# boolsi/boolsi

Measured on AMD Instinct MI355X. Metric: node-state-updates/s, higher is better.
Workload: dtype u32

## Files before the change

### boolsi_amd/csrc/bsx_cascade.cpp

```cpp
#include <cmath>
#include <cstdio>
#include <cstring>

#include "bsx_attract_host.h"

using namespace bsx;

namespace {
constexpr uint64_t kUnresCap = 1ull << 16;
constexpr uint64_t kNearBytes = 1ull << 32;
}

namespace bsx {

static int mirror_slots_for(bsx_handle h, uint32_t* slots_out) {
    const uint64_t entries = (h->cube_mirror ? 2 : 1) * h->journal_states;
    uint32_t slots = 64;
    while (slots < 2 * entries && slots < h->cache_lds_slots) slots *= 2;
    const size_t fixed = h->shmem + 32 + pool_extra_bytes(h->net.nw);
    while (slots < 4 * entries && slots < h->cache_lds_slots && fixed + (size_t)2 * slots * h->cache_stride <= 80 * 1024) slots *= 2;
    h->mirror_slots = *slots_out = std::min(slots, h->cache_lds_slots);
    if (h->knobs.debug) std::fprintf(stderr, "[bsx] mirror: %llu cycle states cached, %u slots\n", (unsigned long long)h->journal_states, *slots_out);
    return BSX_OK;
}

int lean_mirror_slots(bsx_handle h, uint32_t* slots_out, Totals* tot) {
    uint32_t ignored = 0;
    if (!slots_out) slots_out = &ignored;
    if (!h->journal_stale) return mirror_slots_for(h, slots_out);
    unsigned int known = 0;
    HIPCHK(h, hipMemcpy(&known, h->d_cc_count.p, sizeof(known), hipMemcpyDeviceToHost));
    if (tot) ++tot->syncs;
    known = std::min<unsigned int>(known, kCycleJournalCap);
    h->h_journal.resize(known);
    if (known) HIPCHK(h, hipMemcpy(h->h_journal.data(), h->d_cc_journal.p, known * sizeof(CycleRecord), hipMemcpyDeviceToHost));
    uint64_t states = 0;
    uint32_t taken = 0;
    for (const CycleRecord& r : h->h_journal) {
        if (taken >= (uint32_t)kTagAcc + kLdsAcc) break;
        if (!r.ready || r.length == 0 || r.length > kCycleCacheMaxLen) continue;
        states += r.length;
        ++taken;
    }
    h->journal_states = states;
    h->journal_stale = false;
    return mirror_slots_for(h, slots_out);
}

int ensure_mirror_image(bsx_handle h, AttractParams& P, size_t shmem) {
    if (!h->knobs.mirror_image) { P.mirror_image = nullptr; P.mirror_out = nullptr; return BSX_OK; }
    const size_t words = 4 + (size_t)P.cc.lds_slots * (h->cache_stride / 4);
    if (h->image_n != h->h_journal.size() || h->image_slots != P.cc.lds_slots || h->d_mirror.n < words) {
        HIPCHK(h, h->d_mirror.reserve(words));
        AttractParams B = P;
        B.count = 0;
        B.level_in = nullptr;
        B.mirror_image = nullptr;
        B.mirror_out = h->d_mirror.p;
        HIPCHK(h, launch_attract_pool((int)h->net.nw, (int)h->net.k_mux, h->lut_mode, dim3(1), shmem, h->stream, B));
        h->image_n = h->h_journal.size();
        h->image_slots = P.cc.lds_slots;
    }
    P.mirror_image = h->d_mirror.p;
    P.mirror_out = nullptr;
    return BSX_OK;
}

}

namespace {

int order_cube_digits(bsx_handle h, Cube& c) {
    const uint32_t r = (uint32_t)c.rel.size();
    if (r < 2 || r > 64 || !h->knobs.cube_order) return BSX_OK;
    uint64_t need = 0;
    for (uint32_t q = 0; q < r; ++q) need |= 1ull << c.rel[q];
    if (need & ~h->life_valid) {
        LifetimeParams L{};
        L.net = h->net;
        for (int w = 0; w < kMaxW32; ++w) { L.fixmask[w] = h->sp.fixmask[w]; L.fixval[w] = h->sp.fixval[w]; L.base[w] = c.base[w]; L.free_mask[w] = c.free_mask[w]; }
        L.n_digits = r;
        for (uint32_t q = 0; q < r; ++q) L.node[q] = h->model.any[c.rel[q]];
        HIPCHK(h, h->d_life.reserve(64));
        HIPCHK(h, hipMemsetAsync(h->d_life.p, 0, 64 * sizeof(uint32_t), h->stream));
        L.out = h->d_life.p;
        HIPCHK(h, launch_digit_lifetimes((int)h->net.nw, (int)h->net.k_mux, h->lut_mode, h->shmem, h->stream, L));
        uint32_t measured[64];
        HIPCHK(h, hipMemcpyAsync(measured, h->d_life.p, sizeof(measured), hipMemcpyDeviceToHost, h->stream));
        HIPCHK(h, hipStreamSynchronize(h->stream));
        for (uint32_t q = 0; q < r; ++q) h->life_cache[c.rel[q]] = measured[q];
        h->life_valid |= need;
    }
    uint32_t life[64];
    for (uint32_t q = 0; q < r; ++q) life[q] = h->life_cache[c.rel[q]];
// ... 191 lines not shown
            }
        }
        const size_t shmem_here = Q.lower_build ? h->shmem + (size_t)B.slots * h->cache_stride + 32 + pool_lower_extra_bytes(nw) : B.shmem;
        hipStream_t const st = i == 0 ? main_st : tail_st;
        HIPCHK(h, launch_attract_pool((int)nw, (int)h->net.k_mux, h->lut_mode, grid, shmem_here, st, Q));
        if (i == 0) HIPCHK(h, hipEventRecord(ev[1], main_st));
        if (i == 0 && side) HIPCHK(h, hipStreamWaitEvent(tail_st, ev[1], 0));
    }
    if (side) {
        HIPCHK(h, hipEventRecord(ev[2], tail_st));
        slot_busy[slot] = ev[2];
    }
    return BSX_OK;
}

int evaluate_chain(bsx_handle h, const CascadeEnv& env, const CascadeShape& sh, const Chain& ch, MergedTable& pass_table,
                   u128& pass_none, u128& pass_ref, int& verdict, uint32_t& lower_to) {
    const AttractParams& P = env.P;
    Totals& tot = env.tot;
    const uint64_t max_t = env.max_t, max_len = env.max_len;
    const uint32_t nw = h->net.nw, rec_words = nw + 3;
    verdict = kChainOk;
    uint64_t n_entries = 0;
    for (uint32_t i = 0; i < ch.top; ++i) {
        const ChainLevel& l = ch.lv[i];
        const Counters& c = h->ctr_seen[ch.ctr_base + i];
        const uint64_t classes = i == 0 ? 1ull << l.k_bits : n_entries << l.k_bits;
        if (i > 0 && n_entries == 0) break;
        tot.steps_exec += c.steps_exec;
        if (h->knobs.debug)
            std::fprintf(stderr, "[bsx] cube 2^%u (%u digits free) at digit value %llu%s: depth %u%s, %u digits here (%u relevant), %llu classes, %llu near a cycle, %llu unresolved\n",
                         ch.c1.a, ch.c1.n_free, (unsigned long long)ch.c1.d_lo, ch.c1.fix_mask ? " [sub-block]" : "", l.depth, i == 0 ? " (top)" : l.per_parent ? " (per parent)" : "", l.k_bits, l.r_here,
                         (unsigned long long)classes, (unsigned long long)c.near_classes, (unsigned long long)c.straggler_classes);
        if (h->knobs.debug && l.per_parent) {
            const LeafProgram& prog = h->h_leaf[ch.index];
            std::fprintf(stderr, "[bsx] per-parent level: kb %u, %u enumerated rules, %u free rules, m %u\n", prog.kb, prog.n_enum, prog.n_free, prog.m);
        }
        if (c.straggler_overflow) { verdict = kChainGiveUp; return BSX_OK; }
        if (c.near_overflow) { verdict = kChainLower; lower_to = l.depth - 1; return BSX_OK; }
        n_entries = c.near_classes;
        {
            double* seen = h->plan.near_seen[i == 0 ? 0 : 1][std::min<uint32_t>(l.depth, kMaxCubeLevels)];
            seen[0] += (double)classes; seen[1] += (double)c.near_classes;
        }
        const uint32_t us = l.unit_shift;
        merge_cube_counters(pass_table, c, us, nw);
        fold_cube_level(c, us, max_t, pass_none, pass_ref);
        const uint64_t n_unres = c.straggler_classes;
        if (!n_unres) continue;
        if (n_unres > kUnresCap) { verdict = kChainGiveUp; return BSX_OK; }
        std::vector<uint32_t> recs(n_unres * rec_words);
        HIPCHK(h, hipMemcpy(recs.data(), h->d_unres.p + (size_t)(ch.ctr_base + i) * kUnresCap * rec_words, recs.size() * 4, hipMemcpyDeviceToHost));
        ++tot.syncs;
        std::vector<uint32_t> st(n_unres * nw);
        for (uint64_t q = 0; q < n_unres; ++q) std::copy(recs.begin() + q * rec_words, recs.begin() + q * rec_words + nw, st.begin() + q * nw);
        DevBuf<uint32_t> d_states;
        DevBuf<ProblemRec32> d_res;
        HIPCHK(h, d_states.upload(st));
        HIPCHK(h, d_res.alloc(n_unres));
        AttractParams S = P;
        S.sp = l.cube.sp;
        S.sp.tp_origin = 0;
        S.count = n_unres;
        S.states = d_states.p;
        S.per_problem = d_res.p;
        S.max_len = BSX_T_INF;
// ... 244 lines not shown
```

### boolsi_amd/csrc/bsx_device.h

```cpp
#pragma once
#include <cstddef>
#include <stdint.h>

namespace bsx {

constexpr int kWave = 64;
constexpr int kBlock = 512;
constexpr int kWavesPerBlock = kBlock / kWave;
constexpr int kPoolBlockThreads = 768;
constexpr uint32_t kPoolCap = 112;
constexpr uint32_t kPoolSlots = 128;
constexpr uint32_t pool_rec_words(uint32_t nw) { return nw + 4; }
constexpr uint32_t kLowerFoundWords = 256;
constexpr int kMaxW32 = 8;
constexpr int kMaxMuxK = 6;
constexpr int kTableSlots = 64;
constexpr uint32_t kStepLimit = 1u << 30;
constexpr uint64_t kDigestSeed = 0xCBF29CE484222325ull;
constexpr uint64_t kDigestPrime = 0x100000001B3ull;
constexpr uint32_t kMaxDepositRuns = 64;

struct DevNet {
    uint32_t n_nodes;
    uint32_t nw;
// ... 29 lines not shown
    uint64_t first_variant;
};

struct LogRec {
    uint32_t key[kMaxW32];
    uint32_t length;
    uint32_t pad;
    uint64_t count;
    uint64_t sum_l;
    uint64_t sum_l2_lo, sum_l2_hi;
};
static_assert(sizeof(LogRec) == 72, "LogRec layout");

struct ProblemRec32 {
    uint32_t key[kMaxW32];
    uint32_t length;
    uint32_t trajectory_l;
    uint32_t found;
    uint32_t pad;
};

struct alignas(256) Counters {
    unsigned long long cursor;
    unsigned long long steps_ref;
    unsigned long long steps_exec;
    unsigned long long n_none;
    unsigned long long log_cursor;
    unsigned int log_overflow;
    unsigned int step_limit_hits;
    unsigned long long n_stragglers;
    unsigned long long n_cache_resolved;
    unsigned long long straggler_classes;
    unsigned int straggler_overflow;
    unsigned int pad;
    unsigned long long table_inserts;
    unsigned int table_overflow;
    unsigned int near_overflow;
    unsigned long long phase_sum[3];
    unsigned long long phase_max[3];
    unsigned long long acc_cnt[64], acc_sl[64], acc_sl2_lo[64], acc_sl2_hi[64];
    unsigned int acc_len[64];
    unsigned int acc_key[64][kMaxW32];
    unsigned long long fix_cnt[64], fix_sl[64], fix_sl2[64];
    unsigned long long fix_none, fix_ref, fix_capfail;
    unsigned long long near_classes;
    unsigned long long t_first_not, t_last;
    unsigned long long wave_iters;
    unsigned long long service_rounds;
    unsigned long long diag[4];
};

constexpr uint32_t kCycleCacheMaxLen = 64;
constexpr uint32_t kCycleCacheLdsBytes = 16 * 1024;
constexpr uint32_t kCycleJournalCap = 4096;
constexpr uint32_t kCycleClaimSlots = 8192;
constexpr int kTagAcc = 3;
constexpr uint32_t kLdsAcc = 61;
constexpr uint32_t kMergeGroup = 32;
constexpr uint32_t kMergeSlots = 256;
constexpr uint32_t lean_acc_bytes(uint32_t nw) { return (kTagAcc + kLdsAcc) * (8 + 8 + 4 + 4 + 4 * nw) + 16 + kWavesPerBlock * (kMergeSlots + 256); }

struct CycleRecord {
    uint32_t key[kMaxW32];
    uint32_t length;
    uint32_t ready;
};
static_assert(sizeof(CycleRecord) == 40, "CycleRecord layout");

struct CycleCache {
    CycleRecord* journal;
    unsigned int* journal_count;
    unsigned int* claims;
    uint32_t enabled;
    uint32_t lds_slots;
};

struct LevelDesc {
    unsigned long long n_entries;
    unsigned int abort;
    unsigned int pad;
};
constexpr uint32_t kMaxCubeLevels = 16;
constexpr uint32_t kSideStreams = 4;
constexpr uint32_t kMaxChains = 48;
constexpr uint32_t kMaxChainBlocks = 160;
constexpr size_t kLevelDescBytes = 3584;
constexpr size_t kPublishTicketOffset = kLevelDescBytes - 16;
static_assert(sizeof(LevelDesc) * (kMaxChainBlocks + kMaxChains + 1) <= kPublishTicketOffset && kLevelDescBytes % 256 == 0, "descriptor block");

constexpr uint32_t kLeafMaxDeps = 64;
constexpr uint32_t kLeafMaxBits = 14;
constexpr uint32_t kLeafMaxK = 4;
struct LeafDep {
// ... 144 lines not shown
```

### boolsi_amd/csrc/bsx_engine.h

```cpp
#pragma once
#include <hip/hip_runtime.h>

#include <map>
#include <string>
#include <utility>
#include <vector>

#include "bsx.h"
#include "bsx_device.h"
#include "bsx_knobs.h"
#include "bsx_model.h"

namespace bsx {

struct WideHost;

template <typename T>
struct DevBuf {
    T* p = nullptr;
    size_t n = 0;
    DevBuf() = default;
    DevBuf(const DevBuf&) = delete;
    DevBuf& operator=(const DevBuf&) = delete;
    ~DevBuf() { release(); }
// ... 32 lines not shown

    bool have_net = false;
    uint32_t n_nodes = 0, w64 = 0;
    bsx::DevNet net{};
    int lut_mode = 0;
    size_t shmem = 0;
    size_t shmem_attract = 0;

    bool cache_enabled = true;
    int lean_blocks_per_cu = 0;
    bool fast_ok = true;
    bool pool_ok = false;
    size_t cache_stride = 0;
    std::vector<bsx::CycleRecord> h_journal;
    bool journal_stale = true;
    uint32_t mirror_slots = 64;
    uint64_t journal_states = 0;
    bool cube_mirror = false;
    uint32_t fast_steps = 0;
    bool fast_calibrated = false;
    uint32_t cache_lds_slots = 0;
    bsx::DevBuf<bsx::CycleRecord> d_cc_journal;
    bsx::DevBuf<unsigned int> d_cc_claims;
    bsx::DevBuf<unsigned int> d_cc_count;

    bsx::DevBuf<bsx::LogRec> d_log;
    bsx::DevBuf<bsx::LogRec> d_table;
    uint64_t table_slots = 0;
    bool table_dirty = false;
    bsx::DevBuf<uint32_t> d_strag;
    bsx::DevBuf<uint32_t> d_mirror;
    size_t image_n = ~size_t(0);
    uint32_t image_slots = 0;
    bsx::DevBuf<uint32_t> d_near_seg[bsx::kSideStreams];
    bsx::DevBuf<uint32_t> d_near_list[bsx::kSideStreams][2];
    hipStream_t side[bsx::kSideStreams] = {};
    bsx::DevBuf<uint32_t> d_unres;
    bsx::DevBuf<bsx::LeafProgram> d_leaf;
    bsx::LeafProgram* h_leaf = nullptr;
    uint32_t life_cache[64] = {};
    uint64_t life_valid = 0;
    bsx::PlanState plan;
    bsx::DevBuf<uint32_t> d_life;
    bsx::DevBuf<uint32_t> d_lut, d_masks, d_wide_desc, d_wide_preds, d_wide_tt;

    bsx::HostModel model;

    bool have_space = false;
    uint64_t variant_count = 1;
    bool variant_count_saturated = false;
    uint32_t tp_max = 0;
    bsx::DevSpace sp{};
    bsx::DevBuf<uint32_t> d_any, d_fv, d_pv, d_set, d_clr;

    bsx::DevBuf<unsigned char> d_ctr_raw;
    bsx::LevelDesc* d_level = nullptr;
    bsx::Counters* d_ctr = nullptr;
    bsx::Counters* h_ctr = nullptr;
    volatile uint32_t* h_flag = nullptr;
    uint32_t flag_seq = 0;
    hipEvent_t ev_top0 = nullptr, ev_top1 = nullptr;
    std::vector<bsx::Counters> ctr_seen;
    std::vector<hipEvent_t> ev_chain;
    hipStream_t aux[8] = {};
    hipEvent_t aux_done[8] = {};
    bsx::DevBuf<bsx::Counters> d_ctr_multi;
// ... 54 lines not shown
```

### boolsi_amd/csrc/bsx_kernels_common.h

```cpp
#pragma once
#include <hip/hip_runtime.h>
#include <type_traits>
#include "bsx_device.h"

namespace bsx {

__device__ __forceinline__ uint32_t bfi(uint32_t sel, uint32_t a, uint32_t b) {
    uint32_t r;
    asm("v_bfi_b32 %0, %1, %2, %3" : "=v"(r) : "v"(sel), "v"(a), "v"(b));
    return r;
}

#define BSX_KERNARG(Type, name)                                                                          \
    const Type* name = (const Type*)__builtin_amdgcn_kernarg_segment_ptr();                              \
    asm volatile("" : "+s"(name))

__device__ __forceinline__ uint32_t rank_below(uint64_t mask) {
    return __builtin_amdgcn_mbcnt_hi((uint32_t)(mask >> 32), __builtin_amdgcn_mbcnt_lo((uint32_t)mask, 0u));
}

template <int NW>
__device__ __forceinline__ bool eq_words(const uint32_t (&a)[NW], const uint32_t (&b)[NW]) {
    uint32_t d = 0;
#pragma unroll
// ... 286 lines not shown
        else { digit = (uint32_t)(variant & 1); variant >>= 1; }
        const int st = digit_state(range, digit);
        if (st >= 0) { put_bit<NW>(pr.fm, node, 1); put_bit<NW>(pr.fv, node, (uint32_t)st); }
    }
    pr.pv_digits = 0;
    pr.tp = sp.tp_origin;
    for (uint32_t j = 0; j < sp.n_pv; ++j) {
        const uint32_t t = sp.pv[3 * j], range = sp.pv[3 * j + 2];
        uint32_t digit;
        if (range == 3) { digit = (uint32_t)(variant % 3); variant /= 3; }
        else { digit = (uint32_t)(variant & 1); variant >>= 1; }
        pr.pv_digits |= (uint64_t)digit << (2 * j);
        if (digit_state(range, digit) >= 0 && t > pr.tp) pr.tp = t;
    }
}

template <int NW>
__device__ __forceinline__ void apply_perturbations(const DevSpace& sp, uint32_t t, uint64_t pv_digits,
                                                    uint32_t (&s)[NW]) {
    if (t <= sp.tp_origin) {
#pragma unroll
        for (int w = 0; w < NW; ++w)
            s[w] = (s[w] & ~sp.sched_clr[t * NW + w]) | sp.sched_set[t * NW + w];
    }
    for (uint32_t j = 0; j < sp.n_pv; ++j) {
        if (sp.pv[3 * j] == t) {
            const int st = digit_state(sp.pv[3 * j + 2], (uint32_t)(pv_digits >> (2 * j)) & 3u);
            if (st >= 0) put_bit<NW>(s, sp.pv[3 * j + 1], (uint32_t)st);
        }
    }
}

template <int NW, int K, int LM>
__device__ __forceinline__ NetView<NW, K, LM> stage_network(const DevNet& net, uint32_t* smem, uint32_t*& smem_free) {
    constexpr bool LDS_LUT = LM != kLutGlobal;
    NetView<NW, K, LM> nv;
    if constexpr (LDS_LUT) {
        if ((uint32_t)(uintptr_t)(__attribute__((address_space(3))) uint32_t*)smem != 0u) __builtin_trap();
    }
    uint32_t* p = smem;
    uint32_t* smasks = p;
    const uint32_t n_masks = (1u << K) * NW;
    for (uint32_t i = threadIdx.x; i < n_masks; i += blockDim.x) smasks[i] = net.masks[i];
    p += (n_masks + 3u) & ~3u;
    if (LDS_LUT) {
        uint32_t* slut = p;
        const uint4* src = reinterpret_cast<const uint4*>(net.lut);
        uint4* dst = reinterpret_cast<uint4*>(slut);
        const uint32_t n4 = net.lut_words >> 2;
        for (uint32_t i = threadIdx.x; i < n4; i += blockDim.x) dst[i] = src[i];
        p += net.lut_words;
        nv.lut = slut;
    } else {
        nv.lut = net.lut;
    }
    __syncthreads();
    nv.masks = smasks;
    if constexpr (NetView<NW, K, LM>::kMasksInRegs) {
#pragma unroll
        for (int i = 0; i < (1 << K) * NW; ++i) nv.mreg[i] = smasks[i];
    } else {
        nv.mreg[0] = 0;
    }
    nv.n_wide = net.n_wide;
    nv.wide_desc = net.wide_desc;
    nv.wide_preds = net.wide_preds;
    nv.wide_tt = net.wide_tt;
    smem_free = p;
    return nv;
}

__device__ __forceinline__ uint32_t digest_ybit(uint32_t t) { return (t * 0x9E3779B1u) >> 31; }
template <int NW>
__device__ __forceinline__ uint64_t digest_fold_words(uint64_t dg, const uint32_t (&s)[NW], uint32_t w64) {
#pragma unroll
    for (int w = 0; w < (NW + 1) / 2; ++w) {
        uint64_t word = s[2 * w];
        if (2 * w + 1 < NW) word |= (uint64_t)s[2 * w + 1] << 32;
        if ((uint32_t)w < w64) dg = (dg ^ word) * kDigestPrime;
    }
    return dg;
}

__device__ __forceinline__ uint64_t bcast64(uint64_t v, int src_lane) {
    const uint32_t lo = __builtin_amdgcn_readlane((uint32_t)v, src_lane);
    const uint32_t hi = __builtin_amdgcn_readlane((uint32_t)(v >> 32), src_lane);
    return ((uint64_t)hi << 32) | lo;
}

__device__ __forceinline__ unsigned long long wave_sum(unsigned long long v) {
#pragma unroll
    for (int off = 32; off >= 1; off >>= 1) {
        const uint32_t lo = __shfl_xor((uint32_t)v, off, 64);
        const uint32_t hi = __shfl_xor((uint32_t)(v >> 32), off, 64);
        v += ((unsigned long long)hi << 32) | lo;
    }
    return v;
}
__device__ __forceinline__ void wave_atomic_add(unsigned long long* dst, unsigned long long v, int lane) {
    const unsigned long long total = wave_sum(v);
    if (lane == 0 && total) atomicAdd(dst, total);
}
// ... 341 lines not shown
```

### boolsi_amd/csrc/bsx_pool_kernel.h

```cpp
#pragma once
#include "bsx_kernels_common.h"
#include "bsx_leaf.h"

namespace bsx {

constexpr int kPoolBlock = kPoolBlockThreads;
constexpr int kPoolWaves = kPoolBlock / 64;
constexpr uint32_t kPoolGroup = 64;

constexpr int pool_min_waves(int nw) { return nw <= 2 ? 6 : 2; }

#define BSX_RARE_PARAMS(name) BSX_KERNARG(AttractParams, name)

template <int NW>
__device__ __forceinline__ void deposit_runs(const DevSpace& sp, uint64_t d, uint32_t (&s)[NW], uint32_t run_first = 0,
                                             uint32_t run_end = 0xFFFFFFFFu) {
    const uint32_t end = run_end < sp.n_runs ? run_end : sp.n_runs;
    for (uint32_t r = run_first; r < end; ++r) {
        const uint32_t desc = sp.deposit[2 * r], mask = sp.deposit[2 * r + 1];
        const uint32_t piece = ((uint32_t)(d >> (desc & 63u)) & mask) << ((desc >> 16) & 31u);
        const uint32_t word = (desc >> 8) & 7u;
#pragma unroll
        for (int w = 0; w < NW; ++w) s[w] |= (word == (uint32_t)w) ? piece : 0u;
    }
}

template <int NW, int K, int LM, bool CUBE, bool LOWER = false>
__global__ __launch_bounds__(kPoolBlock, pool_min_waves(NW)) void k_attract_pool(const AttractParams P) {
    static_assert(CUBE || !LOWER, "the lower-level build is a cube build");
    extern __shared__ __attribute__((aligned(16))) uint32_t smem[];
    uint32_t* smem_free;
#ifdef BSX_DIAG
    const unsigned long long dbg_t0 = wall_clock64();
#endif
    uint64_t n_items = P.count, chunk_first = P.chunk_first;
    uint32_t chunk = P.chunk;
    if constexpr (CUBE) {
        if (P.level_in) {
            const unsigned long long listed = P.level_in->n_entries;
            n_items = P.level_in->abort ? 0ull : listed << P.entry_shift;
            if constexpr (LOWER) {
                if (P.leaf && n_items) n_items = ((listed + 63ull) & ~63ull) * leaf_parts(P.leaf->m, listed, (uint64_t)gridDim.x * kPoolWaves);
            }
            if (n_items == 0) return;
            const uint64_t n_waves = (uint64_t)gridDim.x * kPoolWaves;
            if (n_items < (1ull << 28)) { chunk_first = ((n_items + n_waves - 1) / n_waves + 63) / 64 * 64; chunk = 0; }
            else { chunk_first = 4096; chunk = 4096; }
            if ((uint64_t)blockIdx.x * chunk_first >= n_items) return;
        }
    }
    if constexpr (CUBE) {
        if (threadIdx.x == 0 && !P.mirror_out) atomicMax(&P.ctr->t_first_not, ~(unsigned long long)wall_clock64());
    }
    const NetView<NW, K, LM> nv = stage_network<NW, K, LM>(P.net, smem, smem_free);
    const uint32_t lane = threadIdx.x & 63, wave = __builtin_amdgcn_readfirstlane(threadIdx.x >> 6);
    const uint32_t tp = P.sp.tp_origin;
    const bool has_warmup = tp != 0;
    const bool counting = CUBE || P.merge >= 2;
    constexpr bool cube = CUBE;
    const int32_t fast_steps = (int32_t)P.fast_steps;
    const uint32_t cmask = P.cc.lds_slots - 1;
    constexpr int S = CacheLayout<NW>::kStride;
    constexpr uint32_t kAccs = (uint32_t)kTagAcc + kLdsAcc;
    constexpr uint32_t R = cube ? NW + 2 : pool_rec_words(NW);
    constexpr uint32_t kCap = cube ? (kPoolCap * pool_rec_words(NW)) / (NW + 2) : kPoolCap;

    uint32_t* lc = smem + (((uint32_t)(smem_free - smem) + 3u) & ~3u);
    const uint32_t lc_words = kCacheHeaderWords + P.cc.lds_slots * S;
    unsigned long long* acc_sl2 = reinterpret_cast<unsigned long long*>(lc + ((lc_words + 1u) & ~1u));
    unsigned long long* acc_sl2h = acc_sl2 + kAccs;
    unsigned long long* acc_sl = acc_sl2h + kAccs;
    unsigned long long* acc_cnt = acc_sl + kAccs;
    uint32_t* lamtab = reinterpret_cast<uint32_t*>(acc_cnt + kAccs);
    uint32_t* keytab = lamtab + kAccs;
    constexpr uint32_t kWaveWords = LOWER ? 0u : kPoolCap * pool_rec_words(NW) + 128 + kPoolSlots / 4;
    constexpr uint32_t kFoundWords = LOWER ? kLowerFoundWords : 0u;
    constexpr uint32_t kLowerCntWords = LOWER ? 2u * kAccs : 0u;
    static_assert(kAccs % 2 == 0 && kWaveWords % 2 == 0, "64-bit LDS atomics need 8-byte aligned tables");
    unsigned long long* wg_ctr = reinterpret_cast<unsigned long long*>(keytab + ((kAccs * NW + 1u) & ~1u));
    uint32_t* midtab = reinterpret_cast<uint32_t*>(wg_ctr + 4);
    uint32_t* wave_base = midtab + 64 * NW + kFoundWords + wave * (kWaveWords + kLowerCntWords);
    typedef volatile uint32_t __attribute__((address_space(3))) lds_vu32;
    typedef volatile uint8_t __attribute__((address_space(3))) lds_vu8;
    lds_vu32* const pool = (lds_vu32*)(__attribute__((address_space(3))) uint32_t*)wave_base;
    lds_vu32* const dd_acc = pool + kPoolCap * pool_rec_words(NW);
    lds_vu8* const dd_ids = (lds_vu8*)(dd_acc + 128);

    uint32_t fm0[NW], fv0[NW];
    uint32_t any_fixed = 0;
#pragma unroll
    for (int w = 0; w < NW; ++w) { fm0[w] = P.sp.fixmask[w]; fv0[w] = P.sp.fixval[w]; any_fixed |= fm0[w]; }
    const bool has_fixed = any_fixed != 0;
    const uint32_t* const image = P.mirror_image;
    if (image) { for (uint32_t i = threadIdx.x; i < lc_words; i += blockDim.x) lc[i] = image[i]; }
    else { for (uint32_t i = threadIdx.x; i < lc_words; i += blockDim.x) lc[i] = 0; }
    for (uint32_t i = threadIdx.x; i < kAccs; i += blockDim.x) { acc_sl2[i] = 0; acc_sl2h[i] = 0; acc_sl[i] = 0; acc_cnt[i] = 0; lamtab[i] = 0; }
    if (threadIdx.x < 4) wg_ctr[threadIdx.x] = 0;
    if constexpr (!LOWER) { dd_acc[2 * lane] = 0; dd_acc[2 * lane + 1] = 0; }
    else { wave_base[lane] = 0; wave_base[64 + lane] = 0; }
    __syncthreads();
    if (!image && threadIdx.x == 0) {
        uint32_t seen = 0, n_states = 0, n_attr = 0;
        cache_pull<NW, K>(P.cc, nv, fm0, fv0, lc, seen, n_states, n_attr, kAccs);
    }
    __syncthreads();
    if (P.mirror_out) {
        for (uint32_t i = threadIdx.x; i < lc_words; i += blockDim.x) P.mirror_out[i] = lc[i];
        return;
    }
    const uint32_t* cbase = lc + kCacheHeaderWords;
    for (uint32_t sl = threadIdx.x; sl < P.cc.lds_slots; sl += blockDim.x) {
        const uint32_t tg = cbase[sl * S + NW] & kTagMask;
        if (tg) {
            lamtab[tg - 1] = cbase[sl * S + NW + 1];
#pragma unroll
            for (int w = 0; w < NW; ++w) keytab[(tg - 1) * NW + w] = cbase[sl * S + NW + 2 + w];
        }
    }
    __syncthreads();
    if constexpr (cube) {
        for (uint32_t i = threadIdx.x; i < 64u; i += blockDim.x) {
            uint32_t m[NW];
#pragma unroll
            for (int w = 0; w < NW; ++w) m[w] = 0;
            deposit_runs<NW>(P.sp, (uint64_t)i << 6, m, 6u, 12u);
#pragma unroll
            for (int w = 0; w < NW; ++w) midtab[i * NW + w] = m[w];
        }
    }
    const uint32_t depth = (cube && P.cube_depth > 1u) ? P.cube_depth : 1u;
    const bool from_entries = cube && P.entries != nullptr;
    if constexpr (cube) {
        if (threadIdx.x == 0) { lc[1] = 0; lc[2] = 0; }
        __syncthreads();
        if (depth == 1u && !has_warmup) {
            constexpr uint32_t kFoundCap = LOWER ? kLowerFoundWords : kCap * R;
            auto inside = [&](uint32_t sl) -> bool {
                const uint32_t* e = cbase + sl * S;
                const uint32_t tw = e[NW];
                if ((tw & kTagMask) == 0 || (tw & kTagRep)) return false;
                uint32_t outside = 0;
#pragma unroll
                for (int w = 0; w < NW; ++w) outside |= (e[w] ^ P.sp.origin[w]) & ~P.cube_free[w];
                return outside == 0;
            };
            lds_vu32* const found0 = (lds_vu32*)(__attribute__((address_space(3))) uint32_t*)(midtab + 64 * NW);
            for (uint32_t sl = threadIdx.x; sl < P.cc.lds_slots; sl += blockDim.x) {
                if (!inside(sl)) continue;
                const uint32_t at = atomicAdd((uint32_t*)(__attribute__((address_space(3))) uint32_t*)&lc[1], 1u);
                if (at < kFoundCap) found0[at] = sl;
            }
            __syncthreads();
            if (threadIdx.x == 0) {
                const uint32_t n_in = lc[1];
                auto add_rep = [&](uint32_t sl) {
                    const uint32_t* e = cbase + sl * S;
                    uint32_t rep[NW], key[NW], differs = 0;
#pragma unroll
                    for (int w = 0; w < NW; ++w) {
                        rep[w] = e[w] & ~P.cube_umask[w];
                        differs |= rep[w] ^ e[w];
                        key[w] = e[NW + 2 + w];
                    }
                    if (differs) cache_insert_lds<NW>(lc, cmask, rep, e[NW + 1], key, (e[NW] & kTagMask) | kTagRep);
                };
                if (n_in <= kFoundCap) {
                    for (uint32_t i = 0; i < n_in; ++i) add_rep(found0[i]);
                } else {
                    for (uint32_t sl = 0; sl < P.cc.lds_slots; ++sl) if (inside(sl)) add_rep(sl);
                }
            }
        }
    }
    __syncthreads();
    const bool t0_lookup = cube && !has_warmup && depth == 1u && __builtin_amdgcn_readfirstlane(lc[1]) != 0;
    uint32_t lane_part[NW];
#pragma unroll
    for (int w = 0; w < NW; ++w) lane_part[w] = 0;
    if constexpr (cube) deposit_runs<NW>(P.sp, (uint64_t)lane, lane_part);
    uint32_t u_hi[NW];
    uint64_t u_hi_tag = ~0ull;
#pragma unroll
    for (int w = 0; w < NW; ++w) u_hi[w] = 0;

    const uint32_t cap_rel = (P.cap_rel_inf || P.max_t - tp >= (kStepLimit / 4)) ? 0xFFFFFFFFu : (uint32_t)(P.max_t - tp);

    using cnt_t = std::conditional_t<CUBE, unsigned long long, uint32_t>;
    uint32_t nexec = 0;
    const uint64_t first_dyn = (uint64_t)gridDim.x * kPoolWaves * chunk_first;
    WaveQueue q{0, 0, chunk != 0 && n_items > first_dyn};
    {
        const uint64_t b = ((uint64_t)wave * gridDim.x + blockIdx.x) * chunk_first;
        if (b < n_items) { q.next = b; q.end = (b + chunk_first < n_items) ? b + chunk_first : n_items; }
    }
    uint32_t head = 0, count = 0;
#ifdef BSX_DIAG
    unsigned long long dbg_iters = 0, dbg_fresh = 0, dbg_fresh_keep = 0, dbg_pool_in = 0, dbg_pool_keep = 0, dbg_merged = 0;
    bool dbg_is_fresh = false;
#endif

    uint32_t ptag = 0;
    auto fresh_state = [&](uint64_t pos, bool lv, uint32_t (&S0)[NW]) {
        if ((pos >> 12) != u_hi_tag) {
            u_hi_tag = pos >> 12;
#pragma unroll
            for (int w = 0; w < NW; ++w) u_hi[w] = P.sp.origin[w];
            deposit_runs<NW>(P.sp, pos & ~0xFFFull, u_hi, 12u);
// ... 595 lines not shown
                if constexpr (NW == 2) {
                    typedef volatile bsx_u32x4 __attribute__((address_space(3))) lds_v4;
                    bsx_u32x4 v;
                    v.x = A[0]; v.y = A[1]; v.z = mlo; v.w = packed;
                    *(lds_v4*)(pool + r) = v;
                } else {
#pragma unroll
                    for (int w = 0; w < NW; ++w) pool[r + w] = A[w];
                    pool[r + NW] = mlo; pool[r + NW + 1] = packed;
                }
            } else if constexpr (NW % 2 == 0) {
                typedef volatile bsx_u32x2 __attribute__((address_space(3))) lds_v2;
                lds_v2* rec = (lds_v2*)(pool + r);
#pragma unroll
                for (int w = 0; w < NW; w += 2) { bsx_u32x2 v; v.x = A[w]; v.y = A[w + 1]; rec[w / 2] = v; }
                bsx_u32x2 b0, b1;
                b0.x = base; b0.y = mlo; b1.x = mhi; b1.y = (uint32_t)t;
                rec[NW / 2] = b0; rec[NW / 2 + 1] = b1;
            } else {
#pragma unroll
                for (int w = 0; w < NW; ++w) pool[r + w] = A[w];
                pool[r + NW] = base; pool[r + NW + 1] = mlo; pool[r + NW + 2] = mhi; pool[r + NW + 3] = (uint32_t)t;
            }
        }
        count += (uint32_t)__popcll(keepers);
        __builtin_amdgcn_fence(__ATOMIC_RELEASE, "wavefront");
        __builtin_amdgcn_wave_barrier();
    }

    __syncthreads();
#ifdef BSX_DIAG
    const unsigned long long dbg_t2 = wall_clock64();
#endif
    static_assert(kAccs == 64, "one lane per accumulator");
    if (wave == 0) {
        const uint32_t a = lane;
        const unsigned long long cn = acc_cnt[a];
        const uint64_t nb = __ballot(cn != 0);
        if (nb) {
            unsigned long long at0 = 0;
            if (!cube && lane == 0) at0 = atomicAdd(&P.ctr->log_cursor, (unsigned long long)__popcll(nb));
            const unsigned long long at = bcast64(at0, 0) + rank_below(nb);
            if (cn) {
                const unsigned long long sl = acc_sl[a];
                if constexpr (cube) {
                    Counters* c = P.ctr;
                    atomicAdd(&c->acc_cnt[a], cn);
                    atomicAdd(&c->acc_sl[a], sl);
                    const unsigned long long lo = acc_sl2[a];
                    const unsigned long long old = atomicAdd(&c->acc_sl2_lo[a], lo);
                    const unsigned long long up = acc_sl2h[a] + ((old + lo < old) ? 1ull : 0ull);
                    if (up) atomicAdd(&c->acc_sl2_hi[a], up);
                    c->acc_len[a] = lamtab[a];
#pragma unroll
                    for (int w = 0; w < NW; ++w) c->acc_key[a][w] = keytab[a * NW + w];
                } else if (at < P.log_cap) {
                    LogRec r;
#pragma unroll
                    for (int w = 0; w < kMaxW32; ++w) r.key[w] = 0;
#pragma unroll
                    for (int w = 0; w < NW; ++w) r.key[w] = keytab[a * NW + w];
                    r.length = lamtab[a]; r.pad = 0; r.count = cn; r.sum_l = sl; r.sum_l2_lo = acc_sl2[a]; r.sum_l2_hi = acc_sl2h[a];
                    P.log[at] = r;
                } else {
                    atomicOr(&P.ctr->log_overflow, 1u);
                }
                atomicAdd(&wg_ctr[2], sl + cn * lamtab[a]);
            }
        }
    }
#ifdef BSX_DIAG
    if (lane == 0) {
        atomicAdd(&P.ctr->wave_iters, dbg_iters); atomicAdd(&P.ctr->service_rounds, dbg_fresh);
        atomicAdd(&P.ctr->diag[0], dbg_fresh_keep); atomicAdd(&P.ctr->diag[1], dbg_pool_in);
        atomicAdd(&P.ctr->diag[2], dbg_pool_keep); atomicAdd(&P.ctr->diag[3], dbg_merged);
    }
    if (threadIdx.x == 0) {
        const unsigned long long dbg_t3 = wall_clock64();
        atomicAdd(&P.ctr->phase_sum[0], dbg_t1 - dbg_t0); atomicMax(&P.ctr->phase_max[0], dbg_t1 - dbg_t0);
        atomicAdd(&P.ctr->phase_sum[1], dbg_t2 - dbg_t1); atomicMax(&P.ctr->phase_max[1], dbg_t2 - dbg_t1);
        atomicAdd(&P.ctr->phase_sum[2], dbg_t3 - dbg_t2); atomicMax(&P.ctr->phase_max[2], dbg_t3 - dbg_t2);
    }
#endif
    {
        const unsigned long long w_exec = wave_sum((unsigned long long)nexec);
        if (lane == 0 && w_exec) atomicAdd(&wg_ctr[3], w_exec);
    }
    __builtin_amdgcn_fence(__ATOMIC_RELEASE, "workgroup");
    __builtin_amdgcn_s_barrier();
    __builtin_amdgcn_fence(__ATOMIC_ACQUIRE, "workgroup");
    if (threadIdx.x == 0) {
        if constexpr (cube) {
            BSX_RARE_PARAMS(Pr);
            if (Pr->level_out) {
                const uint32_t listed = lc[2];
                const uint32_t mine = listed < Pr->near_cap ? listed : (uint32_t)Pr->near_cap;
                lc[1] = mine ? (uint32_t)atomicAdd(&Pr->level_out->n_entries, (unsigned long long)mine) : 0u;
                if (listed) atomicAdd(&P.ctr->near_classes, (unsigned long long)listed);
                if (listed > Pr->near_cap) {
                    atomicOr(&Pr->level_out->abort, 1u);
                    atomicOr(&P.ctr->near_overflow, 1u);
                }
            }
        }
        const unsigned long long ref = wg_ctr[2] + (P.cap_rel_inf ? 0ull : wg_ctr[1] * P.max_t);
        if (ref) atomicAdd(&P.ctr->steps_ref, ref);
        if (wg_ctr[3]) atomicAdd(&P.ctr->steps_exec, wg_ctr[3]);
        if (wg_ctr[0]) atomicAdd(&P.ctr->n_none, wg_ctr[0]);
        if constexpr (cube) atomicMax(&P.ctr->t_last, (unsigned long long)wall_clock64());
    }
    if constexpr (cube) {
        BSX_RARE_PARAMS(Pr);
        if (Pr->level_out) {
            __syncthreads();
            const uint32_t listed = lc[2], base = lc[1];
            const uint64_t words = (uint64_t)(listed < Pr->near_cap ? listed : (uint32_t)Pr->near_cap) * (NW + 1);
            const uint32_t* src = Pr->near + (uint64_t)blockIdx.x * Pr->near_cap * (NW + 1);
            uint32_t* dst = Pr->near_list + (uint64_t)base * (NW + 1);
            for (uint64_t i = threadIdx.x; i < words; i += kPoolBlock) dst[i] = src[i];
        }
    }
}

template <int NW, int K, int LM>
__global__ __launch_bounds__(1024) void k_digit_lifetimes(const LifetimeParams P) {
    extern __shared__ __attribute__((aligned(16))) uint32_t smem[];
    uint32_t* smem_free;
    const NetView<NW, K, LM> nv = stage_network<NW, K, LM>(P.net, smem, smem_free);
    const uint32_t digit = threadIdx.x / kLifeTrials, trial = threadIdx.x % kLifeTrials;
    if (digit >= P.n_digits) return;
    uint32_t fm[NW], fv[NW], x[NW], y[NW];
    uint32_t any_fixed = 0;
    const uint32_t node = P.node[digit];
#pragma unroll
    for (int w = 0; w < NW; ++w) {
        fm[w] = P.fixmask[w]; fv[w] = P.fixval[w]; any_fixed |= fm[w];
        uint32_t rnd = (trial * 0x9E3779B1u + (uint32_t)w * 0x85EBCA6Bu + 0x27D4EB2Fu) * 0xC2B2AE35u;
        rnd ^= rnd >> 15; rnd *= 0x2C1B3C6Du; rnd ^= rnd >> 12;
        const uint32_t bit = ((node >> 5) == (uint32_t)w) ? 1u << (node & 31) : 0u;
        x[w] = (P.base[w] | (trial ? rnd & P.free_mask[w] : 0u)) & ~bit;
        y[w] = x[w] | bit;
    }
    uint32_t t = 0;
    while (t < kLifeSteps && !eq_words<NW>(x, y)) {
        uint32_t nx[NW], ny[NW];
        net_step<NW, K>(nv, x, fm, fv, nx, any_fixed != 0);
        net_step<NW, K>(nv, y, fm, fv, ny, any_fixed != 0);
// ... 113 lines not shown
```

Baseline: 3583 billion.

## Stage whole LDS prologue from a precomputed image and move near-list reservation earlier

The mirror image now holds the full LDS prologue (masks, LUT, cycle cache, accumulators, lamtab, keytab, counters), not just the cache. When an image is present, each workgroup loads it with one batched vector copy instead of staging the network, zeroing accumulators and rebuilding lookup tables, which removes several barriers. The near-list slot reservation atomic moves earlier to wave 1 so the final barrier before the copy-out can go. This adds image-size bookkeeping and depends on the LDS layout matching pool_image_words exactly, which is a correctness risk.

```diff
diff --git a/boolsi_amd/csrc/bsx_cascade.cpp b/boolsi_amd/csrc/bsx_cascade.cpp
--- a/boolsi_amd/csrc/bsx_cascade.cpp
+++ b/boolsi_amd/csrc/bsx_cascade.cpp
@@ -49,8 +49,8 @@
 
 int ensure_mirror_image(bsx_handle h, AttractParams& P, size_t shmem) {
     if (!h->knobs.mirror_image) { P.mirror_image = nullptr; P.mirror_out = nullptr; return BSX_OK; }
-    const size_t words = 4 + (size_t)P.cc.lds_slots * (h->cache_stride / 4);
-    if (h->image_n != h->h_journal.size() || h->image_slots != P.cc.lds_slots || h->d_mirror.n < words) {
+    const size_t words = pool_image_words(h->net.nw, h->net.k_mux, h->lut_mode != 0, h->net.lut_words, P.cc.lds_slots);
+    if (h->image_n != h->h_journal.size() || h->image_slots != P.cc.lds_slots || h->image_words != words || h->d_mirror.n < words) {
         HIPCHK(h, h->d_mirror.reserve(words));
         AttractParams B = P;
         B.count = 0;
@@ -60,6 +60,7 @@
         HIPCHK(h, launch_attract_pool((int)h->net.nw, (int)h->net.k_mux, h->lut_mode, dim3(1), shmem, h->stream, B));
         h->image_n = h->h_journal.size();
         h->image_slots = P.cc.lds_slots;
+        h->image_words = words;
     }
     P.mirror_image = h->d_mirror.p;
     P.mirror_out = nullptr;
@@ -317,6 +318,11 @@
             std::fprintf(stderr, "[bsx] cube 2^%u (%u digits free) at digit value %llu%s: depth %u%s, %u digits here (%u relevant), %llu classes, %llu near a cycle, %llu unresolved\n",
                          ch.c1.a, ch.c1.n_free, (unsigned long long)ch.c1.d_lo, ch.c1.fix_mask ? " [sub-block]" : "", l.depth, i == 0 ? " (top)" : l.per_parent ? " (per parent)" : "", l.k_bits, l.r_here,
                          (unsigned long long)classes, (unsigned long long)c.near_classes, (unsigned long long)c.straggler_classes);
+        if (h->knobs.debug && c.phase_wgs)
+            std::fprintf(stderr, "[bsx]   diag: depth %u, %llu classes, %u workgroups with work; prologue / loop / epilogue, us: mean %.1f / %.1f / %.1f, slowest %.1f / %.1f / %.1f\n",
+                         l.depth, (unsigned long long)classes, c.phase_wgs,
+                         c.phase_sum[0] / 100.0 / c.phase_wgs, c.phase_sum[1] / 100.0 / c.phase_wgs, c.phase_sum[2] / 100.0 / c.phase_wgs,
+                         c.phase_max[0] / 100.0, c.phase_max[1] / 100.0, c.phase_max[2] / 100.0);
         if (h->knobs.debug && l.per_parent) {
             const LeafProgram& prog = h->h_leaf[ch.index];
             std::fprintf(stderr, "[bsx] per-parent level: kb %u, %u enumerated rules, %u free rules, m %u\n", prog.kb, prog.n_enum, prog.n_free, prog.m);
diff --git a/boolsi_amd/csrc/bsx_device.h b/boolsi_amd/csrc/bsx_device.h
--- a/boolsi_amd/csrc/bsx_device.h
+++ b/boolsi_amd/csrc/bsx_device.h
@@ -85,7 +85,7 @@
     unsigned long long n_cache_resolved;
     unsigned long long straggler_classes;
     unsigned int straggler_overflow;
-    unsigned int pad;
+    unsigned int phase_wgs;
     unsigned long long table_inserts;
     unsigned int table_overflow;
     unsigned int near_overflow;
@@ -112,6 +112,18 @@
 constexpr uint32_t kMergeGroup = 32;
 constexpr uint32_t kMergeSlots = 256;
 constexpr uint32_t lean_acc_bytes(uint32_t nw) { return (kTagAcc + kLdsAcc) * (8 + 8 + 4 + 4 + 4 * nw) + 16 + kWavesPerBlock * (kMergeSlots + 256); }
+
+constexpr uint32_t pool_image_words(uint32_t nw, uint32_t k_mux, bool lut_in_lds, uint32_t lut_words, uint32_t lds_slots) {
+    const uint32_t accs = (uint32_t)kTagAcc + kLdsAcc;
+    const uint32_t masks = (((1u << k_mux) * nw) + 3u) & ~3u;
+    const uint32_t lut = lut_in_lds ? lut_words : 0u;
+    const uint32_t mirror = 4u + lds_slots * (((2u * nw + 2u) + 3u) & ~3u);
+    const uint32_t sums = 4u * 2u * accs;
+    const uint32_t lamtab = accs;
+    const uint32_t keytab = (accs * nw + 1u) & ~1u;
+    const uint32_t wg_ctr = 4u * 2u;
+    return (masks + lut + mirror + sums + lamtab + keytab + wg_ctr + 3u) & ~3u;
+}
 
 struct CycleRecord {
     uint32_t key[kMaxW32];
diff --git a/boolsi_amd/csrc/bsx_engine.h b/boolsi_amd/csrc/bsx_engine.h
--- a/boolsi_amd/csrc/bsx_engine.h
+++ b/boolsi_amd/csrc/bsx_engine.h
@@ -88,6 +88,7 @@
     bsx::DevBuf<uint32_t> d_mirror;
     size_t image_n = ~size_t(0);
     uint32_t image_slots = 0;
+    size_t image_words = 0;
     bsx::DevBuf<uint32_t> d_near_seg[bsx::kSideStreams];
     bsx::DevBuf<uint32_t> d_near_list[bsx::kSideStreams][2];
     hipStream_t side[bsx::kSideStreams] = {};
diff --git a/boolsi_amd/csrc/bsx_kernels_common.h b/boolsi_amd/csrc/bsx_kernels_common.h
--- a/boolsi_amd/csrc/bsx_kernels_common.h
+++ b/boolsi_amd/csrc/bsx_kernels_common.h
@@ -342,42 +342,75 @@
 }
 
 template <int NW, int K, int LM>
-__device__ __forceinline__ NetView<NW, K, LM> stage_network(const DevNet& net, uint32_t* smem, uint32_t*& smem_free) {
+__device__ __forceinline__ NetView<NW, K, LM> network_view(const DevNet& net, uint32_t* smem, uint32_t*& smem_free) {
     constexpr bool LDS_LUT = LM != kLutGlobal;
     NetView<NW, K, LM> nv;
     if constexpr (LDS_LUT) {
         if ((uint32_t)(uintptr_t)(__attribute__((address_space(3))) uint32_t*)smem != 0u) __builtin_trap();
     }
     uint32_t* p = smem;
-    uint32_t* smasks = p;
-    const uint32_t n_masks = (1u << K) * NW;
-    for (uint32_t i = threadIdx.x; i < n_masks; i += blockDim.x) smasks[i] = net.masks[i];
-    p += (n_masks + 3u) & ~3u;
+    nv.masks = p;
+    p += (((1u << K) * NW) + 3u) & ~3u;
     if (LDS_LUT) {
-        uint32_t* slut = p;
-        const uint4* src = reinterpret_cast<const uint4*>(net.lut);
-        uint4* dst = reinterpret_cast<uint4*>(slut);
-        const uint32_t n4 = net.lut_words >> 2;
-        for (uint32_t i = threadIdx.x; i < n4; i += blockDim.x) dst[i] = src[i];
+        nv.lut = p;
         p += net.lut_words;
-        nv.lut = slut;
     } else {
         nv.lut = net.lut;
     }
-    __syncthreads();
-    nv.masks = smasks;
-    if constexpr (NetView<NW, K, LM>::kMasksInRegs) {
-#pragma unroll
-        for (int i = 0; i < (1 << K) * NW; ++i) nv.mreg[i] = smasks[i];
-    } else {
-        nv.mreg[0] = 0;
-    }
+    nv.mreg[0] = 0;
     nv.n_wide = net.n_wide;
     nv.wide_desc = net.wide_desc;
     nv.wide_preds = net.wide_preds;
     nv.wide_tt = net.wide_tt;
     smem_free = p;
     return nv;
+}
+
+template <int NW, int K, int LM>
+__device__ __forceinline__ void load_mask_regs(NetView<NW, K, LM>& nv) {
+    if constexpr (NetView<NW, K, LM>::kMasksInRegs) {
+#pragma unroll
+        for (int i = 0; i < (1 << K) * NW; ++i) nv.mreg[i] = nv.masks[i];
+    }
+}
+
+template <int NW, int K, int LM>
+__device__ __forceinline__ NetView<NW, K, LM> stage_network(const DevNet& net, uint32_t* smem, uint32_t*& smem_free) {
+    constexpr bool LDS_LUT = LM != kLutGlobal;
+    NetView<NW, K, LM> nv = network_view<NW, K, LM>(net, smem, smem_free);
+    uint32_t* smasks = smem;
+    const uint32_t n_masks = (1u << K) * NW;
+    for (uint32_t i = threadIdx.x; i < n_masks; i += blockDim.x) smasks[i] = net.masks[i];
+    if (LDS_LUT) {
+        const uint4* src = reinterpret_cast<const uint4*>(net.lut);
+        uint4* dst = reinterpret_cast<uint4*>(smem + ((n_masks + 3u) & ~3u));
+        const uint32_t n4 = net.lut_words >> 2;
+        for (uint32_t i = threadIdx.x; i < n4; i += blockDim.x) dst[i] = src[i];
+    }
+    __syncthreads();
+    load_mask_regs<NW, K, LM>(nv);
+    return nv;
+}
+
+constexpr int kImageLoadsPerRound = 4;
+__device__ __forceinline__ void copy_table_image(uint32_t* smem, const uint32_t* image, uint32_t n4) {
+    const bsx_u32x4* src = reinterpret_cast<const bsx_u32x4*>(__builtin_assume_aligned(image, 16));
+    bsx_u32x4* dst = reinterpret_cast<bsx_u32x4*>(__builtin_assume_aligned(smem, 16));
+    static_assert(kImageLoadsPerRound == 4, "the round's loads are pinned by name below");
+    for (uint32_t first = threadIdx.x; first < n4; first += kImageLoadsPerRound * blockDim.x) {
+        bsx_u32x4 v[kImageLoadsPerRound];
+#pragma unroll
+        for (int j = 0; j < kImageLoadsPerRound; ++j) {
+            const uint32_t i = first + (uint32_t)j * blockDim.x;
+            v[j] = src[i < n4 ? i : n4 - 1u];
+        }
+        asm volatile("" : "+v"(v[0]), "+v"(v[1]), "+v"(v[2]), "+v"(v[3]));
+#pragma unroll
+        for (int j = 0; j < kImageLoadsPerRound; ++j) {
+            const uint32_t i = first + (uint32_t)j * blockDim.x;
+            if (i < n4) dst[i] = v[j];
+        }
+    }
 }
 
 __device__ __forceinline__ uint32_t digest_ybit(uint32_t t) { return (t * 0x9E3779B1u) >> 31; }
diff --git a/boolsi_amd/csrc/bsx_pool_kernel.h b/boolsi_amd/csrc/bsx_pool_kernel.h
--- a/boolsi_amd/csrc/bsx_pool_kernel.h
+++ b/boolsi_amd/csrc/bsx_pool_kernel.h
@@ -52,7 +52,8 @@
     if constexpr (CUBE) {
         if (threadIdx.x == 0 && !P.mirror_out) atomicMax(&P.ctr->t_first_not, ~(unsigned long long)wall_clock64());
     }
-    const NetView<NW, K, LM> nv = stage_network<NW, K, LM>(P.net, smem, smem_free);
+    const uint32_t* const image = P.mirror_image;
+    NetView<NW, K, LM> nv = image ? network_view<NW, K, LM>(P.net, smem, smem_free) : stage_network<NW, K, LM>(P.net, smem, smem_free);
     const uint32_t lane = threadIdx.x & 63, wave = __builtin_amdgcn_readfirstlane(threadIdx.x >> 6);
     const uint32_t tp = P.sp.tp_origin;
     const bool has_warmup = tp != 0;
@@ -91,49 +92,64 @@
 #pragma unroll
     for (int w = 0; w < NW; ++w) { fm0[w] = P.sp.fixmask[w]; fv0[w] = P.sp.fixval[w]; any_fixed |= fm0[w]; }
     const bool has_fixed = any_fixed != 0;
-    const uint32_t* const image = P.mirror_image;
-    if (image) { for (uint32_t i = threadIdx.x; i < lc_words; i += blockDim.x) lc[i] = image[i]; }
-    else { for (uint32_t i = threadIdx.x; i < lc_words; i += blockDim.x) lc[i] = 0; }
-    for (uint32_t i = threadIdx.x; i < kAccs; i += blockDim.x) { acc_sl2[i] = 0; acc_sl2h[i] = 0; acc_sl[i] = 0; acc_cnt[i] = 0; lamtab[i] = 0; }
-    if (threadIdx.x < 4) wg_ctr[threadIdx.x] = 0;
-    if constexpr (!LOWER) { dd_acc[2 * lane] = 0; dd_acc[2 * lane + 1] = 0; }
-    else { wave_base[lane] = 0; wave_base[64 + lane] = 0; }
-    __syncthreads();
-    if (!image && threadIdx.x == 0) {
-        uint32_t seen = 0, n_states = 0, n_attr = 0;
-        cache_pull<NW, K>(P.cc, nv, fm0, fv0, lc, seen, n_states, n_attr, kAccs);
-    }
-    __syncthreads();
-    if (P.mirror_out) {
-        for (uint32_t i = threadIdx.x; i < lc_words; i += blockDim.x) P.mirror_out[i] = lc[i];
-        return;
-    }
     const uint32_t* cbase = lc + kCacheHeaderWords;
-    for (uint32_t sl = threadIdx.x; sl < P.cc.lds_slots; sl += blockDim.x) {
-        const uint32_t tg = cbase[sl * S + NW] & kTagMask;
-        if (tg) {
-            lamtab[tg - 1] = cbase[sl * S + NW + 1];
-#pragma unroll
-            for (int w = 0; w < NW; ++w) keytab[(tg - 1) * NW + w] = cbase[sl * S + NW + 2 + w];
-        }
-    }
-    __syncthreads();
-    if constexpr (cube) {
-        for (uint32_t i = threadIdx.x; i < 64u; i += blockDim.x) {
-            uint32_t m[NW];
-#pragma unroll
-            for (int w = 0; w < NW; ++w) m[w] = 0;
-            deposit_runs<NW>(P.sp, (uint64_t)i << 6, m, 6u, 12u);
-#pragma unroll
-            for (int w = 0; w < NW; ++w) midtab[i * NW + w] = m[w];
+    auto launch_tables = [&]() {
+        if constexpr (!LOWER) { dd_acc[2 * lane] = 0; dd_acc[2 * lane + 1] = 0; }
+        else { wave_base[lane] = 0; wave_base[64 + lane] = 0; }
+        if constexpr (cube) {
+            for (uint32_t i = threadIdx.x; i < 64u; i += blockDim.x) {
+                uint32_t m[NW];
+#pragma unroll
+                for (int w = 0; w < NW; ++w) m[w] = 0;
+                deposit_runs<NW>(P.sp, (uint64_t)i << 6, m, 6u, 12u);
+#pragma unroll
+                for (int w = 0; w < NW; ++w) midtab[i * NW + w] = m[w];
+            }
+        }
+    };
+    if (image) {
+        copy_table_image(smem, image, pool_image_words(NW, K, LM != kLutGlobal, P.net.lut_words, P.cc.lds_slots) >> 2);
+        launch_tables();
+        __syncthreads();
+        load_mask_regs<NW, K, LM>(nv);
+    } else {
+        for (uint32_t i = threadIdx.x; i < lc_words; i += blockDim.x) lc[i] = 0;
+        for (uint32_t i = threadIdx.x; i < kAccs; i += blockDim.x) { acc_sl2[i] = 0; acc_sl2h[i] = 0; acc_sl[i] = 0; acc_cnt[i] = 0; lamtab[i] = 0; }
+        if (threadIdx.x < 4) wg_ctr[threadIdx.x] = 0;
+        if (P.mirror_out) for (uint32_t i = threadIdx.x; i < ((kAccs * NW + 1u) & ~1u); i += blockDim.x) keytab[i] = 0;
+        __syncthreads();
+        if (threadIdx.x == 0) {
+            uint32_t seen = 0, n_states = 0, n_attr = 0;
+            cache_pull<NW, K>(P.cc, nv, fm0, fv0, lc, seen, n_states, n_attr, kAccs);
+        }
+        __syncthreads();
+        for (uint32_t sl = threadIdx.x; sl < P.cc.lds_slots; sl += blockDim.x) {
+            const uint32_t tg = cbase[sl * S + NW] & kTagMask;
+            if (tg) {
+                lamtab[tg - 1] = cbase[sl * S + NW + 1];
+#pragma unroll
+                for (int w = 0; w < NW; ++w) keytab[(tg - 1) * NW + w] = cbase[sl * S + NW + 2 + w];
+            }
+        }
+        __syncthreads();
+        if (P.mirror_out) {
+            const uint32_t n4 = pool_image_words(NW, K, LM != kLutGlobal, P.net.lut_words, P.cc.lds_slots) >> 2;
+            const uint4* src = reinterpret_cast<const uint4*>(smem);
+            uint4* dst = reinterpret_cast<uint4*>(P.mirror_out);
+            for (uint32_t i = threadIdx.x; i < n4; i += blockDim.x) dst[i] = src[i];
+            return;
+        }
+        launch_tables();
+        if constexpr (cube) {
+            if (threadIdx.x == 0) { lc[1] = 0; lc[2] = 0; }
+            __syncthreads();
         }
     }
     const uint32_t depth = (cube && P.cube_depth > 1u) ? P.cube_depth : 1u;
     const bool from_entries = cube && P.entries != nullptr;
+    const bool rep_search = cube && depth == 1u && !has_warmup;
     if constexpr (cube) {
-        if (threadIdx.x == 0) { lc[1] = 0; lc[2] = 0; }
-        __syncthreads();
-        if (depth == 1u && !has_warmup) {
+        if (rep_search) {
             constexpr uint32_t kFoundCap = LOWER ? kLowerFoundWords : kCap * R;
             auto inside = [&](uint32_t sl) -> bool {
                 const uint32_t* e = cbase + sl * S;
@@ -172,7 +188,7 @@
             }
         }
     }
-    __syncthreads();
+    if (!image || rep_search) __syncthreads();
     const bool t0_lookup = cube && !has_warmup && depth == 1u && __builtin_amdgcn_readfirstlane(lc[1]) != 0;
     uint32_t lane_part[NW];
 #pragma unroll
@@ -834,6 +850,19 @@
 #ifdef BSX_DIAG
     const unsigned long long dbg_t2 = wall_clock64();
 #endif
+    static_assert(kPoolWaves >= 2, "the span is reserved by wave 1");
+    if constexpr (cube) {
+        if (threadIdx.x == 64) {
+            BSX_RARE_PARAMS(Pr);
+            LevelDesc* const out = Pr->level_out;
+            const uint64_t cap = Pr->near_cap;
+            if (out) {
+                const uint32_t listed = lc[2];
+                const uint32_t mine = listed < cap ? listed : (uint32_t)cap;
+                lc[1] = mine ? (uint32_t)atomicAdd(&out->n_entries, (unsigned long long)mine) : 0u;
+            }
+        }
+    }
     static_assert(kAccs == 64, "one lane per accumulator");
     if (wave == 0) {
         const uint32_t a = lane;
@@ -882,6 +911,7 @@
         atomicAdd(&P.ctr->phase_sum[0], dbg_t1 - dbg_t0); atomicMax(&P.ctr->phase_max[0], dbg_t1 - dbg_t0);
         atomicAdd(&P.ctr->phase_sum[1], dbg_t2 - dbg_t1); atomicMax(&P.ctr->phase_max[1], dbg_t2 - dbg_t1);
         atomicAdd(&P.ctr->phase_sum[2], dbg_t3 - dbg_t2); atomicMax(&P.ctr->phase_max[2], dbg_t3 - dbg_t2);
+        atomicAdd(&P.ctr->phase_wgs, 1u);
     }
 #endif
     {
@@ -896,8 +926,6 @@
             BSX_RARE_PARAMS(Pr);
             if (Pr->level_out) {
                 const uint32_t listed = lc[2];
-                const uint32_t mine = listed < Pr->near_cap ? listed : (uint32_t)Pr->near_cap;
-                lc[1] = mine ? (uint32_t)atomicAdd(&Pr->level_out->n_entries, (unsigned long long)mine) : 0u;
                 if (listed) atomicAdd(&P.ctr->near_classes, (unsigned long long)listed);
                 if (listed > Pr->near_cap) {
                     atomicOr(&Pr->level_out->abort, 1u);
@@ -914,7 +942,6 @@
     if constexpr (cube) {
         BSX_RARE_PARAMS(Pr);
         if (Pr->level_out) {
-            __syncthreads();
             const uint32_t listed = lc[2], base = lc[1];
             const uint64_t words = (uint64_t)(listed < Pr->near_cap ? listed : (uint32_t)Pr->near_cap) * (NW + 1);
             const uint32_t* src = Pr->near + (uint64_t)blockIdx.x * Pr->near_cap * (NW + 1);
```

Measured after the change: 2591 billion. 27.7% lower.
